# Alan-404/Conformer

Measured on AMD Instinct MI355X. Metric: encoder audio-frames/sec (B=32,T=1000,d=512,L=16), higher is better.
Workload: dtype f32; 1 GPU; cfg2 Conformer-L Encoder.forward: B=32/GPU, T=1000 mel frames (T'=249), d=512, 16 blocks, 8 heads, k=31, fp32, eval, random-init weights, batch-sharded replicas; per_gpu_batch=32, mel_frames=1000

## Files before the change

### conformer_amd/csrc/conv2_wino_f32.hip

```cpp
#include <algorithm>
#include <utility>

#include "gemm_shared.h"

namespace {

#define WINO_MFMA_SLICE(FA, FB)                                                                             \
    _Pragma("unroll") for (int e = 0; e < 4; ++e)                                                           \
    _Pragma("unroll") for (int mt = 0; mt < TM; ++mt)                                                       \
    _Pragma("unroll") for (int nt = 0; nt < TN; ++nt)                                                       \
        acc[mt][nt] = __builtin_amdgcn_mfma_f32_32x32x2f32(FB[nt][e], FA[mt][e], acc[mt][nt], 0, 0, 0)

template <typename Fn, int... I>
__device__ __forceinline__ void static_for_seq(Fn& f, std::integer_sequence<int, I...>) {
    (f(std::integral_constant<int, I>{}), ...);
}
template <int N, typename Fn>
__device__ __forceinline__ void static_for(Fn&& f) {
    static_for_seq(f, std::make_integer_sequence<int, N>{});
}

__host__ __device__ constexpr int wino_nt(int a) { return a == 1 ? 1 : 2; }
__host__ __device__ constexpr int wino_terms(int p) { return wino_nt(p / 3) * wino_nt(p % 3); }

struct WinoArgs {
    const float* h1; const float* w; float* planes;
    int64_t M;
    unsigned h1_bytes;
    int T1, F1, C, TI, TJ;
    unsigned tiles_m, tiles_n;
    unsigned grp_blk[4];
};


template <int ST, int SF>
__device__ __forceinline__ void wino_tile(const WinoArgs& g, int p, int64_t m0, int n0, float* lds) {
    constexpr int BM = 256, BN = 256, WN = 4, TM = 4, TN = 2, BK = 16, LDSR = BK + 4, NT = ST * SF, SPC = 2 * NT;
    constexpr int NPX = (ST == 2 ? 2 : 1) * (SF == 2 ? 2 : 1);
    float* As = lds;
    float* Bs = lds + 2 * BM * LDSR;
    const int a = p / 3, b = p - 3 * (p / 3);
    const int sg_t = a >> 1, sg_f = b >> 1;

    const int tid = threadIdx.x, lane = tid & 63;
    const int wave = __builtin_amdgcn_readfirstlane(tid >> 6);
    const int wr = wave / WN, wc = wave % WN;
    const int li = lane & 31, hf = lane >> 5;

    constexpr int CPR = BK / 4, RPP = 512 / CPR, PA = BM / RPP, PB = BN / RPP;
    const int chunk = tid & (CPR - 1), srow = tid / CPR;
    unsigned row_off[PA];
    const int64_t pos_per_b = (int64_t)g.TI * g.TJ;
#pragma unroll
    for (int i = 0; i < PA; ++i) {
        int64_t m = m0 + srow + RPP * i;
        if (m >= g.M) m = g.M - 1;
        const int64_t bb = m / pos_per_b;
        const int r = (int)(m - bb * pos_per_b);
        const int ib = r / g.TJ, jb = r - ib * g.TJ;
        row_off[i] = (unsigned)((((bb * g.T1 + 4 * ib) * g.F1 + 4 * jb) * (int64_t)g.C + chunk * 4) * 4);
    }
    const __amdgpu_buffer_rsrc_t h1_rsrc = __builtin_amdgcn_make_buffer_rsrc(const_cast<float*>(g.h1), (short)0, (int)g.h1_bytes, 0x00020000);
    const unsigned pix_t[3] = {(unsigned)((ST == 2 ? 4 * sg_t : 2) * g.F1 * g.C * 4), (unsigned)(2 * g.F1 * g.C * 4),
                               (unsigned)((1 + 2 * sg_t) * g.F1 * g.C * 4)};
    const unsigned pix_f[3] = {(unsigned)((SF == 2 ? 4 * sg_f : 2) * g.C * 4), (unsigned)(2 * g.C * 4), (unsigned)((1 + 2 * sg_f) * g.C * 4)};
    int64_t woff = 0;
    for (int q = 0; q < p; ++q) woff += wino_terms(q);
    const int K = NT * g.C;
    const __amdgpu_buffer_rsrc_t w_rsrc = __builtin_amdgcn_make_buffer_rsrc(const_cast<float*>(g.w + woff * g.C * g.C), (short)0,
                                                                            K * g.C * 4, 0x00020000);
    unsigned w_off[PB];
#pragma unroll
    for (int i = 0; i < PB; ++i) w_off[i] = (unsigned)(((n0 + srow + RPP * i) * K + chunk * 4) * 4);

    f32x4 raw[PA][NPX], rb[PB];
    auto load_tile = [&](auto U_, int c32, int half) __attribute__((always_inline)) {
        constexpr int U = decltype(U_)::value, UT = U / SF, UF = U % SF;
        constexpr int NXT = (ST == 2 && UT == 0) ? 2 : 1, NYF = (SF == 2 && UF == 0) ? 2 : 1;
        constexpr int X1 = ST == 2 ? (UT == 0 ? 0 : 2) : 0, Y1 = SF == 2 ? (UF == 0 ? 0 : 2) : 0;
        const unsigned ci4 = (unsigned)(32 * c32 + 16 * half) * 4;
#pragma unroll
        for (int x = 0; x < NXT; ++x)
#pragma unroll
            for (int y = 0; y < NYF; ++y) {
                const unsigned po = pix_t[X1 + x] + pix_f[Y1 + y] + ci4;
#pragma unroll
                for (int i = 0; i < PA; ++i)
                    raw[i][x * NYF + y] = __builtin_bit_cast(f32x4, __builtin_amdgcn_raw_buffer_load_b128(h1_rsrc, row_off[i] + po, 0, 0));
            }
        const unsigned k4 = (unsigned)(NT * 32 * c32 + 32 * U + 16 * half) * 4;
#pragma unroll
        for (int i = 0; i < PB; ++i) rb[i] = __builtin_bit_cast(f32x4, __builtin_amdgcn_raw_buffer_load_b128(w_rsrc, w_off[i] + k4, 0, 0));
    };
    auto store_tile = [&](auto U_, int buf) __attribute__((always_inline)) {
        constexpr int U = decltype(U_)::value, UT = U / SF, UF = U % SF;
        constexpr int NXT = (ST == 2 && UT == 0) ? 2 : 1, NYF = (SF == 2 && UF == 0) ? 2 : 1;
#pragma unroll
        for (int i = 0; i < PA; ++i) {
            const f32x4* px = raw[i];
            f32x4 v;
            if constexpr (NXT == 2 && NYF == 2) v = (px[0] - px[1]) - (px[2] - px[3]);
            else if constexpr (NXT * NYF == 2) v = px[0] - px[1];
            else v = px[0];
            *reinterpret_cast<f32x4*>(As + (buf * BM + srow + RPP * i) * LDSR + chunk * 4) = v;
        }
#pragma unroll
        for (int i = 0; i < PB; ++i)
            *reinterpret_cast<f32x4*>(Bs + (buf * BN + srow + RPP * i) * LDSR + chunk * 4) = rb[i];
    };

    f32x16 acc[TM][TN];
#pragma unroll
    for (int i = 0; i < TM; ++i)
#pragma unroll
        for (int j = 0; j < TN; ++j)
#pragma unroll
            for (int r = 0; r < 16; ++r) acc[i][j][r] = 0.f;

    const int a_row = wr * (BM / 2) + li, b_row = wc * (BN / WN) + li;
    f32x4 fa0[TM], fb0[TN], fa1[TM], fb1[TN];
    auto read_frags = [&](f32x4 (&fa)[TM], f32x4 (&fb)[TN], int buf, int c) __attribute__((always_inline)) {
#pragma unroll
        for (int t = 0; t < TM; ++t)
            fa[t] = *reinterpret_cast<const f32x4*>(As + (buf * BM + a_row + 32 * t) * LDSR + 8 * c + 4 * hf);
#pragma unroll
        for (int t = 0; t < TN; ++t)
            fb[t] = *reinterpret_cast<const f32x4*>(Bs + (buf * BN + b_row + 32 * t) * LDSR + 8 * c + 4 * hf);
    };

    const int nch = g.C / 32;
    load_tile(std::integral_constant<int, 0>{}, 0, 0);
    store_tile(std::integral_constant<int, 0>{}, 0);
    load_tile(std::integral_constant<int, 0>{}, 0, 1);
    __syncthreads();
    read_frags(fa0, fb0, 0, 0);
    for (int c32 = 0; c32 < nch; ++c32) {
        static_for<SPC>([&](auto S_) __attribute__((always_inline)) {
            constexpr int S = decltype(S_)::value;
            constexpr int S1 = (S + 1) % SPC, S2 = (S + 2) % SPC;
            const int cur = S & 1;
            const bool more = S + 1 < SPC || c32 + 1 < nch;
            read_frags(fa1, fb1, cur, 1);
            __builtin_amdgcn_sched_barrier(0);
            WINO_MFMA_SLICE(fa0, fb0);
            __builtin_amdgcn_sched_barrier(0);
            if (more) store_tile(std::integral_constant<int, S1 / 2>{}, cur ^ 1);
            load_tile(std::integral_constant<int, S2 / 2>{}, S + 2 < SPC ? c32 : min(c32 + 1, nch - 1), S2 & 1);
            __syncthreads();
            if (more) read_frags(fa0, fb0, cur ^ 1, 0);
            __builtin_amdgcn_sched_barrier(0);
            WINO_MFMA_SLICE(fa1, fb1);
            __builtin_amdgcn_sched_barrier(0);
        });
    }

    __syncthreads();
    GemmArgs ge{};
    ge.C = g.planes + (int64_t)p * g.M * g.C;
    ge.M = g.M; ge.N = g.C; ge.K = K; ge.ldc = g.C; ge.alpha = 1.f;
    gemm_epilogue_rows<BM, BN, EPI_BIAS, TM, TN, 2, false, EPF_INFER | EPF_NO_BIAS, WN>(ge, acc, m0, n0, wr, wc, lane,
                                                                                        lds + wave * 32 * (32 * TN + 4));
}

__global__ __launch_bounds__(512, 2) void conv2_wino_gemm_kernel(const WinoArgs g) {
    constexpr int LDS_STAGE = 2 * (256 + 256) * 20;
    static_assert(8 * 32 * (32 * 2 + 4) <= LDS_STAGE, "the row-major epilogue scratch must fit the staging buffers");
    __shared__ __attribute__((aligned(16))) float lds[LDS_STAGE];
    const unsigned bid = blockIdx.x;
    const int grp = bid < g.grp_blk[1] ? 0 : (bid < g.grp_blk[2] ? 1 : 2);
    const unsigned npat = grp == 2 ? 1u : 4u;
    const unsigned ntile = npat * g.tiles_m * g.tiles_n;
    const unsigned local = bid - g.grp_blk[grp], per_xcd = (g.grp_blk[grp + 1] - g.grp_blk[grp]) / 8;
    const unsigned tile = (local & 7u) * per_xcd + (local >> 3);
    if (tile >= ntile) return;
    const unsigned tn = tile % g.tiles_n, rest = tile / g.tiles_n;
    const unsigned pi = rest % npat, tm = rest / npat;
    const int p = (int)(((grp == 0 ? 0x8620u : grp == 1 ? 0x5371u : 0x4u) >> (4 * pi)) & 15u);
    const int64_t m0 = (int64_t)tm * 256;
    const int n0 = (int)tn * 256;
    const int nta = wino_nt(p / 3), ntb = wino_nt(p % 3);
    if (nta == 2 && ntb == 2) wino_tile<2, 2>(g, p, m0, n0, lds);
    else if (nta == 2) wino_tile<2, 1>(g, p, m0, n0, lds);
    else if (ntb == 2) wino_tile<1, 2>(g, p, m0, n0, lds);
    else wino_tile<1, 1>(g, p, m0, n0, lds);
}

__global__ __launch_bounds__(256) void conv2_wino_combine_kernel(const float* __restrict__ planes, const float* __restrict__ b2,
                                                                 float* __restrict__ h2, int64_t M, int T2, int F2, int TI,
                                                                 int TJ, int C) {
    const int c4n = C / 4;
    const int64_t idx = (int64_t)blockIdx.x * blockDim.x + threadIdx.x;
    if (idx >= M * c4n) return;
    const int64_t m = idx / c4n;
    const int c = (int)(idx - m * c4n) * 4;
    const int64_t per_b = (int64_t)TI * TJ;
    const int64_t bb = m / per_b;
    const int r = (int)(m - bb * per_b);
    const int ib = r / TJ, jb = r - ib * TJ;
    const int64_t plane = M * (int64_t)C;
    f32x4 P[9];
#pragma unroll
    for (int q = 0; q < 9; ++q) P[q] = __builtin_nontemporal_load(reinterpret_cast<const f32x4*>(planes + q * plane + m * C + c));
    const f32x4 bias = *reinterpret_cast<const f32x4*>(b2 + c);
#pragma unroll
    for (int rt = 0; rt < 2; ++rt) {
        const int t2 = 2 * ib + rt;
        if (t2 >= T2) continue;
        const f32x4 u0 = P[3 * rt + 0] + P[3 * rt + 1], u1 = P[3 * rt + 1] + P[3 * rt + 2];
        const f32x4 v0 = P[3 * rt + 3] + P[3 * rt + 4], v1 = P[3 * rt + 4] + P[3 * rt + 5];
#pragma unroll
        for (int s = 0; s < 2; ++s) {
            const int f2 = 2 * jb + s;
            if (f2 >= F2) continue;
            const f32x4 y = (s == 0 ? u0 + v0 : u1 + v1) + bias;
            f32x4 o;
#pragma unroll
            for (int e = 0; e < 4; ++e) o[e] = fmaxf(y[e], 0.f);
            *reinterpret_cast<f32x4*>(h2 + (((bb * T2 + t2) * F2) + f2) * (int64_t)C + c) = o;
        }
    }
}

__global__ __launch_bounds__(256) void pack_conv2_wino_kernel(const float* __restrict__ w2, float* __restrict__ wp, int C) {
    const int p = blockIdx.y, nt = wino_terms(p);
    const int64_t idx = (int64_t)blockIdx.x * blockDim.x + threadIdx.x;
    const int64_t K = (int64_t)nt * C;
    if (idx >= K * C) return;
    const int64_t co = idx / K;
    const int k = (int)(idx - co * K);
    const int c32 = k / (32 * nt), rem = k - c32 * 32 * nt, u = rem / 32, ci = 32 * c32 + (rem & 31);
    int64_t off = 0;
    for (int q = 0; q < p; ++q) off += wino_terms(q);
    const int a = p / 3, b = p % 3, sfn = wino_nt(b);
    const int ut = u / sfn, uf = u % sfn;
    auto taps = [](int pat, int term, int (&tp)[2]) {
        if (pat == 1) { tp[0] = 0; tp[1] = 2; return 2; }
        tp[0] = term == 0 ? 2 * (pat >> 1) : 1;
        return 1;
    };
    int tt[2], tf[2];
    const int ntt = taps(a, ut, tt), ntf = taps(b, uf, tf);
    double s = 0.0;
    const float* wc = w2 + (co * C + ci) * 9;
    for (int x = 0; x < ntt; ++x)
        for (int y = 0; y < ntf; ++y) s += (double)wc[tf[y] * 3 + tt[x]];
    wp[off * C * C + idx] = (float)s;
}

}

extern "C" int64_t cfm_conv2_wino_plane_elems(int B, int F1, int T1, int C) {
    if (B <= 0 || F1 < 3 || T1 < 3 || C <= 0) return 0;
    const int64_t TI = ((T1 - 1) / 2 + 1) / 2, TJ = ((F1 - 1) / 2 + 1) / 2;
    return 9 * (int64_t)B * TI * TJ * C;
}

extern "C" int cfm_pack_conv2_wino_weight_f32(const float* w2, float* wp, int C, cfm_stream_t stream) {
    CFM_REQUIRE(w2 && wp, CFM_ERR_NULL);
    CFM_REQUIRE(C > 0 && C % 32 == 0, CFM_ERR_BAD_SHAPE);
    const int64_t most = 4 * (int64_t)C * C;
    hipLaunchKernelGGL(pack_conv2_wino_kernel, dim3((unsigned)((most + 255) / 256), 9), dim3(256), 0,
                       static_cast<hipStream_t>(stream), w2, wp, C);
    return cfm_launch_status();
}

extern "C" int cfm_subsample_conv2_wino_relu_f32(const float* h1, const float* wp, const float* b2, float* planes, float* h2,
                                                 int B, int F1, int T1, int C, cfm_stream_t stream) {
    CFM_REQUIRE(h1 && wp && b2 && planes && h2, CFM_ERR_NULL);
    CFM_REQUIRE(B > 0 && F1 >= 3 && T1 >= 3, CFM_ERR_BAD_SHAPE);
    CFM_REQUIRE(C > 0 && C % 256 == 0, CFM_ERR_UNSUPPORTED);
    CFM_REQUIRE(CFM_ALIGNED16(h1) && CFM_ALIGNED16(wp) && CFM_ALIGNED16(b2) && CFM_ALIGNED16(planes) && CFM_ALIGNED16(h2),
                CFM_ERR_ALIGN);
    const int64_t utt_bytes = (int64_t)T1 * F1 * C * 4, limit = (1LL << 32) - (1LL << 26);
    CFM_REQUIRE(utt_bytes <= limit && 5LL * F1 * C * 4 < (1LL << 26), CFM_ERR_UNSUPPORTED);
    const int T2 = (T1 - 1) / 2, F2 = (F1 - 1) / 2;
    WinoArgs g{};
    g.w = wp;
    g.T1 = T1; g.F1 = F1; g.C = C; g.TI = (T2 + 1) / 2; g.TJ = (F2 + 1) / 2;
    g.tiles_n = (unsigned)(C / 256);
    const int64_t per_b = (int64_t)g.TI * g.TJ;
    const int group = (int)std::min<int64_t>(B, limit / utt_bytes);
    hipStream_t s = static_cast<hipStream_t>(stream);
    for (int b0 = 0; b0 < B; b0 += group) {
        const int nb = std::min(group, B - b0);
        g.h1 = h1 + b0 * (utt_bytes / 4);
        g.h1_bytes = (unsigned)(nb * utt_bytes);
        g.M = nb * per_b;
        g.planes = planes + 9 * (b0 * per_b) * C;
        g.tiles_m = (unsigned)((g.M + 255) / 256);
        const unsigned group_n[3] = {4, 4, 1};
        g.grp_blk[0] = 0;
        for (int q = 0; q < 3; ++q) g.grp_blk[q + 1] = g.grp_blk[q] + (group_n[q] * g.tiles_m * g.tiles_n + 7) / 8 * 8;
        hipLaunchKernelGGL(conv2_wino_gemm_kernel, dim3(g.grp_blk[3]), dim3(512), 0, s, g);
        int st = cfm_launch_status();
        if (st) return st;
        const int64_t threads = g.M * (C / 4);
        hipLaunchKernelGGL(conv2_wino_combine_kernel, dim3((unsigned)((threads + 255) / 256)), dim3(256), 0, s, g.planes, b2,
                           h2 + (int64_t)b0 * T2 * F2 * C, g.M, T2, F2, g.TI, g.TJ, C);
        st = cfm_launch_status();
        if (st) return st;
    }
    return 0;
}
```

Baseline: 1.665 million audio-frames/sec.

## Skip dead Winograd tile rows for odd output extents per pattern

When the subsampled output size is odd in time or frequency, the Winograd patterns touching the last tile row/column produce contributions that are never used. The GEMM now sizes each pattern's M to exclude those positions, schedules tiles per pattern with a sorted segment table, and the combine kernel reindexes the compacted planes and zero-fills the missing terms. It also moves per-row offsets into the buffer-load soffset argument to save registers. This adds tile-mapping logic in the kernel prologue and only trims a small fraction of the subsampling conv work, which itself is a small part of the encoder.

New measurement: 1.696 million audio-frames/sec, median of 6. 1.02x the previous value.

```diff
diff --git a/conformer_amd/csrc/conv2_wino_f32.hip b/conformer_amd/csrc/conv2_wino_f32.hip
--- a/conformer_amd/csrc/conv2_wino_f32.hip
+++ b/conformer_amd/csrc/conv2_wino_f32.hip
@@ -27,9 +27,12 @@
     const float* h1; const float* w; float* planes;
     int64_t M;
     unsigned h1_bytes;
-    int T1, F1, C, TI, TJ;
-    unsigned tiles_m, tiles_n;
+    int T1, F1, C, TI, TJ, nb;
+    int odd_t, odd_f;
+    unsigned tiles_n;
     unsigned grp_blk[4];
+    unsigned grp_tm[3][4];
+    unsigned grp_pat[3];
 };
 
 
@@ -50,14 +53,15 @@
     constexpr int CPR = BK / 4, RPP = 512 / CPR, PA = BM / RPP, PB = BN / RPP;
     const int chunk = tid & (CPR - 1), srow = tid / CPR;
     unsigned row_off[PA];
-    const int64_t pos_per_b = (int64_t)g.TI * g.TJ;
+    const int TJp = g.TJ - (b == 2 ? g.odd_f : 0);
+    const int64_t pos_per_b = (int64_t)(g.TI - (a == 2 ? g.odd_t : 0)) * TJp, Mp = g.nb * pos_per_b;
 #pragma unroll
     for (int i = 0; i < PA; ++i) {
         int64_t m = m0 + srow + RPP * i;
-        if (m >= g.M) m = g.M - 1;
+        if (m >= Mp) m = Mp - 1;
         const int64_t bb = m / pos_per_b;
         const int r = (int)(m - bb * pos_per_b);
-        const int ib = r / g.TJ, jb = r - ib * g.TJ;
+        const int ib = r / TJp, jb = r - ib * TJp;
         row_off[i] = (unsigned)((((bb * g.T1 + 4 * ib) * g.F1 + 4 * jb) * (int64_t)g.C + chunk * 4) * 4);
     }
     const __amdgpu_buffer_rsrc_t h1_rsrc = __builtin_amdgcn_make_buffer_rsrc(const_cast<float*>(g.h1), (short)0, (int)g.h1_bytes, 0x00020000);
@@ -69,9 +73,7 @@
     const int K = NT * g.C;
     const __amdgpu_buffer_rsrc_t w_rsrc = __builtin_amdgcn_make_buffer_rsrc(const_cast<float*>(g.w + woff * g.C * g.C), (short)0,
                                                                             K * g.C * 4, 0x00020000);
-    unsigned w_off[PB];
-#pragma unroll
-    for (int i = 0; i < PB; ++i) w_off[i] = (unsigned)(((n0 + srow + RPP * i) * K + chunk * 4) * 4);
+    const unsigned w_off = (unsigned)(((n0 + srow) * K + chunk * 4) * 4), w_step = (unsigned)(RPP * K * 4);
 
     f32x4 raw[PA][NPX], rb[PB];
     auto load_tile = [&](auto U_, int c32, int half) __attribute__((always_inline)) {
@@ -86,11 +88,11 @@
                 const unsigned po = pix_t[X1 + x] + pix_f[Y1 + y] + ci4;
 #pragma unroll
                 for (int i = 0; i < PA; ++i)
-                    raw[i][x * NYF + y] = __builtin_bit_cast(f32x4, __builtin_amdgcn_raw_buffer_load_b128(h1_rsrc, row_off[i] + po, 0, 0));
+                    raw[i][x * NYF + y] = __builtin_bit_cast(f32x4, __builtin_amdgcn_raw_buffer_load_b128(h1_rsrc, row_off[i], po, 0));
             }
         const unsigned k4 = (unsigned)(NT * 32 * c32 + 32 * U + 16 * half) * 4;
 #pragma unroll
-        for (int i = 0; i < PB; ++i) rb[i] = __builtin_bit_cast(f32x4, __builtin_amdgcn_raw_buffer_load_b128(w_rsrc, w_off[i] + k4, 0, 0));
+        for (int i = 0; i < PB; ++i) rb[i] = __builtin_bit_cast(f32x4, __builtin_amdgcn_raw_buffer_load_b128(w_rsrc, w_off, k4 + w_step * i, 0));
     };
     auto store_tile = [&](auto U_, int buf) __attribute__((always_inline)) {
         constexpr int U = decltype(U_)::value, UT = U / SF, UF = U % SF;
@@ -157,7 +159,7 @@
     __syncthreads();
     GemmArgs ge{};
     ge.C = g.planes + (int64_t)p * g.M * g.C;
-    ge.M = g.M; ge.N = g.C; ge.K = K; ge.ldc = g.C; ge.alpha = 1.f;
+    ge.M = Mp; ge.N = g.C; ge.K = K; ge.ldc = g.C; ge.alpha = 1.f;
     gemm_epilogue_rows<BM, BN, EPI_BIAS, TM, TN, 2, false, EPF_INFER | EPF_NO_BIAS, WN>(ge, acc, m0, n0, wr, wc, lane,
                                                                                         lds + wave * 32 * (32 * TN + 4));
 }
@@ -168,14 +170,19 @@
     __shared__ __attribute__((aligned(16))) float lds[LDS_STAGE];
     const unsigned bid = blockIdx.x;
     const int grp = bid < g.grp_blk[1] ? 0 : (bid < g.grp_blk[2] ? 1 : 2);
-    const unsigned npat = grp == 2 ? 1u : 4u;
-    const unsigned ntile = npat * g.tiles_m * g.tiles_n;
     const unsigned local = bid - g.grp_blk[grp], per_xcd = (g.grp_blk[grp + 1] - g.grp_blk[grp]) / 8;
-    const unsigned tile = (local & 7u) * per_xcd + (local >> 3);
-    if (tile >= ntile) return;
+    unsigned tile = (local & 7u) * per_xcd + (local >> 3);
+    unsigned k = 0, lo = 0;
+    for (; k < 4; ++k) {
+        const unsigned seg = (g.grp_tm[grp][k] - lo) * (4 - k) * g.tiles_n;
+        if (tile < seg) break;
+        tile -= seg;
+        lo = g.grp_tm[grp][k];
+    }
+    if (k == 4) return;
     const unsigned tn = tile % g.tiles_n, rest = tile / g.tiles_n;
-    const unsigned pi = rest % npat, tm = rest / npat;
-    const int p = (int)(((grp == 0 ? 0x8620u : grp == 1 ? 0x5371u : 0x4u) >> (4 * pi)) & 15u);
+    const unsigned pi = k + rest % (4 - k), tm = lo + rest / (4 - k);
+    const int p = (int)((g.grp_pat[grp] >> (4 * pi)) & 15u);
     const int64_t m0 = (int64_t)tm * 256;
     const int n0 = (int)tn * 256;
     const int nta = wino_nt(p / 3), ntb = wino_nt(p % 3);
@@ -198,9 +205,16 @@
     const int r = (int)(m - bb * per_b);
     const int ib = r / TJ, jb = r - ib * TJ;
     const int64_t plane = M * (int64_t)C;
+    const int TIs = TI - (T2 & 1), TJs = TJ - (F2 & 1);
     f32x4 P[9];
 #pragma unroll
-    for (int q = 0; q < 9; ++q) P[q] = __builtin_nontemporal_load(reinterpret_cast<const f32x4*>(planes + q * plane + m * C + c));
+    for (int q = 0; q < 9; ++q) {
+        const bool st = q / 3 == 2, sf = q % 3 == 2;
+        const int64_t mq = (bb * (st ? TIs : TI) + ib) * (sf ? TJs : TJ) + jb;
+        P[q] = f32x4{0.f, 0.f, 0.f, 0.f};
+        if ((!st || ib < TIs) && (!sf || jb < TJs))
+            P[q] = __builtin_nontemporal_load(reinterpret_cast<const f32x4*>(planes + q * plane + mq * C + c));
+    }
     const f32x4 bias = *reinterpret_cast<const f32x4*>(b2 + c);
 #pragma unroll
     for (int rt = 0; rt < 2; ++rt) {
@@ -277,6 +291,7 @@
     WinoArgs g{};
     g.w = wp;
     g.T1 = T1; g.F1 = F1; g.C = C; g.TI = (T2 + 1) / 2; g.TJ = (F2 + 1) / 2;
+    g.odd_t = T2 & 1; g.odd_f = F2 & 1;
     g.tiles_n = (unsigned)(C / 256);
     const int64_t per_b = (int64_t)g.TI * g.TJ;
     const int group = (int)std::min<int64_t>(B, limit / utt_bytes);
@@ -286,11 +301,26 @@
         g.h1 = h1 + b0 * (utt_bytes / 4);
         g.h1_bytes = (unsigned)(nb * utt_bytes);
         g.M = nb * per_b;
+        g.nb = nb;
         g.planes = planes + 9 * (b0 * per_b) * C;
-        g.tiles_m = (unsigned)((g.M + 255) / 256);
-        const unsigned group_n[3] = {4, 4, 1};
+        static const int group_pat[3][4] = {{0, 2, 6, 8}, {1, 7, 3, 5}, {-1, -1, -1, 4}};
         g.grp_blk[0] = 0;
-        for (int q = 0; q < 3; ++q) g.grp_blk[q + 1] = g.grp_blk[q] + (group_n[q] * g.tiles_m * g.tiles_n + 7) / 8 * 8;
+        for (int q = 0; q < 3; ++q) {
+            int pat[4];
+            unsigned tm[4], total = 0;
+            for (int i = 0; i < 4; ++i) {
+                const int p = group_pat[q][i];
+                const int64_t Mp = p < 0 ? 0 : (int64_t)nb * (g.TI - (p / 3 == 2 ? g.odd_t : 0)) * (g.TJ - (p % 3 == 2 ? g.odd_f : 0));
+                const unsigned t = (unsigned)((Mp + 255) / 256);
+                int j = i;
+                for (; j > 0 && tm[j - 1] > t; --j) { tm[j] = tm[j - 1]; pat[j] = pat[j - 1]; }
+                tm[j] = t; pat[j] = p < 0 ? 0 : p;
+                total += t;
+            }
+            g.grp_pat[q] = 0;
+            for (int i = 0; i < 4; ++i) { g.grp_tm[q][i] = tm[i]; g.grp_pat[q] |= (unsigned)pat[i] << (4 * i); }
+            g.grp_blk[q + 1] = g.grp_blk[q] + (total * g.tiles_n + 7) / 8 * 8;
+        }
         hipLaunchKernelGGL(conv2_wino_gemm_kernel, dim3(g.grp_blk[3]), dim3(512), 0, s, g);
         int st = cfm_launch_status();
         if (st) return st;
```
